# HaokunChen245/FedDAT

Measured on AMD Instinct MI355X. Metric: VQA samples/sec, ViLT-B/32 dual-adapter local step, higher is better.
Workload: dtype fp16; 1 GPU; configs[1] with fp16 operands (BASELINE.json's configs[1] string says bf16: same operand width and MFMA rate; the bf16 step is in other_operand_format with --full): ViLT-B/32 FedDAT, 1 client per MI355X, fp16 MFMA operands (dynamic loss scale, GradScaler semantics on the device, initial 2^14), fp32 accumulate / masters, batch=32/client, 384x384 synthetic + 40-token questions, MKD on; batch_per_client=32, seq_len=185, clients=1, hip_graph=True, ranks=1, hetero_steps=False

## Files before the change

feddat_amd/csrc/adapter_wgrad.hip:

```cpp
#include "common.hip.h"

namespace {

constexpr int H = 768, R = 48, NRT = 3, CW = 64;
constexpr int NCH = H / CW;
constexpr int NBLK = 10;
constexpr int PSTRIDE = R * H + R + H;

__device__ __forceinline__ void split_bf16x2(const float (&x)[8], tbf16x8& head, tbf16x8& rest) {
    typedef unsigned int u32x4_t __attribute__((ext_vector_type(4)));
    head = cvt8_tbf16(f32x4{x[0], x[1], x[2], x[3]}, f32x4{x[4], x[5], x[6], x[7]});
    const u32x4_t hp = __builtin_bit_cast(u32x4_t, head);
    float r[8];
#pragma unroll
    for (int k = 0; k < 4; ++k) {
        r[2 * k] = x[2 * k] - __uint_as_float(hp[k] << 16);
        r[2 * k + 1] = x[2 * k + 1] - __uint_as_float(hp[k] & 0xffff0000u);
    }
    rest = cvt8_tbf16(f32x4{r[0], r[1], r[2], r[3]}, f32x4{r[4], r[5], r[6], r[7]});
}

struct WgradLaunch {
    feddat_wgrad_seg seg[2];
    float* partials;
    int nseg;
};

__global__ __launch_bounds__(256, 2) void wgrad_kernel(WgradLaunch L) {
    __shared__ __attribute__((aligned(16))) float red[3][64][NRT * 4 * 4 + 4];
    const int lane = threadIdx.x & 63;
    const int wave = __builtin_amdgcn_readfirstlane(threadIdx.x >> 6);
    const int g = lane >> 4, i16 = lane & 15;
    const int blk = blockIdx.x, chunk = blockIdx.y;
    const int prob = blockIdx.z;
    const feddat_wgrad_seg& sg = L.seg[prob >> 1];
    const bool up = prob & 1;
    const float* big = up ? sg.dy : sg.x;
    const float* sm = up ? sg.z : sg.dz;
    float unscale = sg.grad_unscale != 0.0f ? sg.grad_unscale : 1.0f;
    if (sg.grad_unscale_dev) unscale *= *sg.grad_unscale_dev;
    const float alpha = (up ? sg.scale : 1.0f) * unscale;
    const int T = sg.rows;
    int tps = (T + NBLK * 4 - 1) / (NBLK * 4);
    tps = (tps + 7) & ~7;
    const int t_begin = (blk * 4 + wave) * tps;
    const int t_end = min(T, t_begin + tps);
    const int c0 = chunk * CW;

    f32x4 acc[NRT][4];
#pragma unroll
    for (int rt = 0; rt < NRT; ++rt)
#pragma unroll
        for (int v = 0; v < 4; ++v) acc[rt][v] = f32x4{0.f, 0.f, 0.f, 0.f};
    f32x4 bsum = {0.f, 0.f, 0.f, 0.f};
    float ssum[NRT] = {0.f, 0.f, 0.f};
    f32x4 braw[8];
    float sraw[8][NRT];
    const int su = NRT * i16;
    auto load_round = [&](int t0, f32x4 (&bq)[8], float (&sq)[8][NRT]) {
#pragma unroll
        for (int e = 0; e < 8; ++e) {
            const int t = t0 + 8 * g + e;
            const int tc = t < t_end ? t : 0;
            bq[e] = *reinterpret_cast<const f32x4*>(big + (size_t)tc * H + c0 + 4 * i16);
            const float* sp = sm + (size_t)tc * R + su;
#pragma unroll
            for (int rt = 0; rt < NRT; ++rt) sq[e][rt] = sp[rt];
        }
    };
    load_round(t_begin, braw, sraw);
    for (int t0 = t_begin; t0 < t_end; t0 += 32) {
        f32x4 bnext[8];
        float snext[8][NRT];
        load_round(t0 + 32, bnext, snext);
#pragma unroll
        for (int e = 0; e < 8; ++e) {
            if (t0 + 8 * g + e >= t_end) {
                braw[e] = f32x4{0.f, 0.f, 0.f, 0.f};
#pragma unroll
                for (int rt = 0; rt < NRT; ++rt) sraw[e][rt] = 0.f;
            }
            bsum = bsum + braw[e];
#pragma unroll
            for (int rt = 0; rt < NRT; ++rt) ssum[rt] += sraw[e][rt];
        }
        tbf16x8 sh[NRT], sl[NRT];
#pragma unroll
        for (int rt = 0; rt < NRT; ++rt) {
            float x[8];
#pragma unroll
            for (int e = 0; e < 8; ++e) x[e] = sraw[e][rt];
            split_bf16x2(x, sh[rt], sl[rt]);
        }
#pragma unroll
        for (int v = 0; v < 4; ++v) {
            float x[8];
#pragma unroll
            for (int e = 0; e < 8; ++e) x[e] = braw[e][v];
            tbf16x8 bh, bl;
            split_bf16x2(x, bh, bl);
#pragma unroll
            for (int rt = 0; rt < NRT; ++rt) {
                acc[rt][v] = mfma16x32_tbf16(sl[rt], bl, acc[rt][v]);
                acc[rt][v] = mfma16x32_tbf16(sl[rt], bh, acc[rt][v]);
                acc[rt][v] = mfma16x32_tbf16(sh[rt], bl, acc[rt][v]);
                acc[rt][v] = mfma16x32_tbf16(sh[rt], bh, acc[rt][v]);
            }
        }
#pragma unroll
        for (int e = 0; e < 8; ++e) {
            braw[e] = bnext[e];
#pragma unroll
            for (int rt = 0; rt < NRT; ++rt) sraw[e][rt] = snext[e][rt];
        }
    }
#pragma unroll
    for (int v = 0; v < 4; ++v) {
        bsum[v] += __shfl_xor(bsum[v], 16, 64);
        bsum[v] += __shfl_xor(bsum[v], 32, 64);
    }
#pragma unroll
    for (int rt = 0; rt < NRT; ++rt) {
        ssum[rt] += __shfl_xor(ssum[rt], 16, 64);
        ssum[rt] += __shfl_xor(ssum[rt], 32, 64);
    }
    if (wave > 0) {
        float* dst = red[wave - 1][lane];
#pragma unroll
        for (int rt = 0; rt < NRT; ++rt)
#pragma unroll
            for (int v = 0; v < 4; ++v) *reinterpret_cast<f32x4*>(dst + (rt * 4 + v) * 4) = acc[rt][v];
        if (g == 0) *reinterpret_cast<f32x4*>(dst + NRT * 16) = bsum;
    }
    __shared__ float red_s[3][NRT][16];
    if (wave > 0 && g == 0) {
#pragma unroll
        for (int rt = 0; rt < NRT; ++rt) red_s[wave - 1][rt][i16] = ssum[rt];
    }
    __syncthreads();
    if (wave != 0) return;
#pragma unroll
    for (int w = 0; w < 3; ++w) {
        const float* src = red[w][lane];
#pragma unroll
        for (int rt = 0; rt < NRT; ++rt)
#pragma unroll
            for (int v = 0; v < 4; ++v) acc[rt][v] = acc[rt][v] + *reinterpret_cast<const f32x4*>(src + (rt * 4 + v) * 4);
        if (g == 0) {
            bsum = bsum + *reinterpret_cast<const f32x4*>(src + NRT * 16);
#pragma unroll
            for (int rt = 0; rt < NRT; ++rt) ssum[rt] += red_s[w][rt][i16];
        }
    }
    float* P = L.partials + ((size_t)prob * NBLK + blk) * PSTRIDE;
#pragma unroll
    for (int rt = 0; rt < NRT; ++rt)
#pragma unroll
        for (int e = 0; e < 4; ++e) {
            const int r = NRT * (4 * g + e) + rt;
            f32x4 o = {alpha * acc[rt][0][e], alpha * acc[rt][1][e], alpha * acc[rt][2][e], alpha * acc[rt][3][e]};
            *reinterpret_cast<f32x4*>(P + (size_t)r * H + c0 + 4 * i16) = o;
        }
    if (g == 0) {
        f32x4 o = {alpha * bsum[0], alpha * bsum[1], alpha * bsum[2], alpha * bsum[3]};
        *reinterpret_cast<f32x4*>(P + R * H + R + c0 + 4 * i16) = o;
        if (chunk == 0) {
#pragma unroll
            for (int rt = 0; rt < NRT; ++rt) P[R * H + NRT * i16 + rt] = unscale * ssum[rt];
        }
    }
}

constexpr int RED_T = 384, RED_UC = 32;
constexpr int RED_UT = H / RED_UC;
constexpr int RED_DQ = (R * H + R) / 4;
constexpr int RED_DB = (RED_DQ + RED_T - 1) / RED_T;
constexpr int RED_BLOCKS = RED_UT + RED_DB + 1;
constexpr int RED_LD = R + 4;
static_assert(R * RED_UC == 4 * RED_T && H % RED_UC == 0 && (R * H) % 4 == 0 && R % 4 == 0 && H / 4 <= RED_T, "reduce tiling");

__device__ __forceinline__ f32x4 wgrad_sum_partials(const float* __restrict__ p0) {
    f32x4 p[NBLK];
#pragma unroll
    for (int b = 0; b < NBLK; ++b) p[b] = *reinterpret_cast<const f32x4*>(p0 + (size_t)b * PSTRIDE);
    f32x4 s = {0.f, 0.f, 0.f, 0.f};
#pragma unroll
    for (int b = 0; b < NBLK; ++b) s = s + p[b];
    return s;
}
__device__ __forceinline__ bool fd_nonfinite4(const f32x4 v) {
    return fd_nonfinite(v[0]) || fd_nonfinite(v[1]) || fd_nonfinite(v[2]) || fd_nonfinite(v[3]);
}

__device__ __forceinline__ bool wgrad_reduce_block(const float* __restrict__ partials, float* __restrict__ gl, int seg) {
    __shared__ __attribute__((aligned(16))) float tile[RED_UC * RED_LD];
    const float* Pd = partials + (size_t)(2 * seg) * NBLK * PSTRIDE;
    const float* Pu = partials + (size_t)(2 * seg + 1) * NBLK * PSTRIDE;
    const int blk = blockIdx.x, q = threadIdx.x;
    if (blk < RED_UT) {
        const int c0 = blk * RED_UC, r = q / (RED_UC / 4), cq = q % (RED_UC / 4);
        const f32x4 su = wgrad_sum_partials(Pu + (size_t)r * H + c0 + 4 * cq);
#pragma unroll
        for (int e = 0; e < 4; ++e) tile[(4 * cq + e) * RED_LD + r] = su[e];
        __syncthreads();
        const int c = q / (R / 4), r4 = 4 * (q % (R / 4));
        const f32x4 o = *reinterpret_cast<const f32x4*>(tile + c * RED_LD + r4);
        *reinterpret_cast<f32x4*>(gl + R * H + R + (size_t)(c0 + c) * R + r4) = o;
        return fd_nonfinite4(o);
    }
    if (blk < RED_UT + RED_DB) {
        const int i = ((blk - RED_UT) * RED_T + q) * 4;
        if (i >= R * H + R) return false;
        const f32x4 sd = wgrad_sum_partials(Pd + i);
        *reinterpret_cast<f32x4*>(gl + i) = sd;
        return fd_nonfinite4(sd);
    }
    if (q >= H / 4) return false;
    const f32x4 su = wgrad_sum_partials(Pu + R * H + R + 4 * q);
    *reinterpret_cast<f32x4*>(gl + R * H + R + H * R + 4 * q) = su;
    return fd_nonfinite4(su);
}

__global__ __launch_bounds__(RED_T) void wgrad_reduce_kernel(WgradLaunch L) {
    wgrad_reduce_block(L.partials, L.seg[blockIdx.y].grad, blockIdx.y);
}

struct WgradReduceBatch {
    float* const* grads;
    const float* partials;
    long stride;
    int nseg;
    int* nonfinite;
};
__global__ __launch_bounds__(RED_T) void wgrad_reduce_batched_kernel(WgradReduceBatch B) {
    const bool bad =
        wgrad_reduce_block(B.partials + (size_t)blockIdx.z * B.stride, B.grads[blockIdx.z * B.nseg + blockIdx.y], blockIdx.y);
    if (B.nonfinite && __ballot(bad) != 0 && (threadIdx.x & 63) == 0) atomicOr(B.nonfinite + blockIdx.y, 1);
}

}

extern "C" long feddat_adapter_wgrad_workspace_elems(int nseg) { return (long)nseg * 2 * NBLK * PSTRIDE; }

static int wgrad_launch(const feddat_wgrad_seg* segs, int nseg, float* partials, long partials_elems, int Hd, int r,
                        bool reduce_now, hipStream_t stream) {
    FD_CHECK_ARG(segs && nseg >= 1 && nseg <= 2 && partials && Hd == H && r == R);
    FD_CHECK_ARG(partials_elems >= (long)nseg * 2 * NBLK * PSTRIDE);
    WgradLaunch L;
    L.nseg = nseg;
    L.partials = partials;
    for (int s = 0; s < nseg; ++s) {
        FD_CHECK_ARG(segs[s].x && segs[s].dy && segs[s].z && segs[s].dz && segs[s].grad && segs[s].rows > 0);
        FD_CHECK_ARG(!reduce_now || (((uintptr_t)segs[s].grad | (uintptr_t)partials) & 15) == 0);
        L.seg[s] = segs[s];
    }
    if (nseg == 1) L.seg[1] = L.seg[0];
    hipLaunchKernelGGL(wgrad_kernel, dim3(NBLK, NCH, 2 * nseg), dim3(256), 0, stream, L);
    if (reduce_now) hipLaunchKernelGGL(wgrad_reduce_kernel, dim3(RED_BLOCKS, nseg), dim3(RED_T), 0, stream, L);
    FD_LAUNCH_RET();
}

extern "C" int feddat_adapter_wgrad(const feddat_wgrad_seg* segs, int nseg, float* partials, long partials_elems,
                                    int Hd, int r, hipStream_t stream) {
    return wgrad_launch(segs, nseg, partials, partials_elems, Hd, r, true, stream);
}

extern "C" int feddat_adapter_wgrad_partial(const feddat_wgrad_seg* segs, int nseg, float* partials, long partials_elems,
                                            int Hd, int r, hipStream_t stream) {
    return wgrad_launch(segs, nseg, partials, partials_elems, Hd, r, false, stream);
}

extern "C" int feddat_adapter_wgrad_reduce(float* const* grads_dev, int n, int nseg, const float* partials,
                                           long partials_stride, hipStream_t stream) {
    FD_CHECK_ARG(grads_dev && partials && n > 0 && n <= 65535 && nseg >= 1 && nseg <= 2);
    FD_CHECK_ARG(partials_stride >= (long)nseg * 2 * NBLK * PSTRIDE);
    FD_CHECK_ARG(((uintptr_t)partials & 15) == 0 && partials_stride % 4 == 0);
    hipLaunchKernelGGL(wgrad_reduce_batched_kernel, dim3(RED_BLOCKS, nseg, n), dim3(RED_T), 0, stream,
                       WgradReduceBatch{grads_dev, partials, partials_stride, nseg, nullptr});
    FD_LAUNCH_RET();
}

extern "C" int feddat_adapter_wgrad_reduce_checked(float* const* grads_dev, int n, int nseg, const float* partials,
                                                   long partials_stride, int* nonfinite, hipStream_t stream) {
    FD_CHECK_ARG(grads_dev && partials && n > 0 && n <= 65535 && nseg >= 1 && nseg <= 2 && nonfinite);
    FD_CHECK_ARG(partials_stride >= (long)nseg * 2 * NBLK * PSTRIDE);
    FD_CHECK_ARG(((uintptr_t)partials & 15) == 0 && partials_stride % 4 == 0);
    hipLaunchKernelGGL(wgrad_reduce_batched_kernel, dim3(RED_BLOCKS, nseg, n), dim3(RED_T), 0, stream,
                       WgradReduceBatch{grads_dev, partials, partials_stride, nseg, nonfinite});
    FD_LAUNCH_RET();
}
```

Before: 4894 samples/s.

## Software-pipeline adapter wgrad loads and spread block reduction across all waves

Restructures the adapter weight-gradient kernel's main loop into ping-pong register buffers. Big-operand loads for the next round are issued up front, and the small-operand loads are deferred until after the current split. Bf16 splitting of the next column tile is interleaved with the current tile's MFMAs using sched_barriers. The cross-wave reduction now has all four waves write to shared memory, and waves 1-3 each reduce and store one rank tile while wave 0 handles the bias and sum terms. This removes the serial single-wave epilogue. It also loads the device unscale factor early and disables fp contraction to keep the arithmetic identical. The costs are more registers and shared memory, which may hurt occupancy at 2 blocks per CU.

Measured after the change: 4907 samples/s (median of 6 runs). No clear change (+0.3%).

```diff
diff --git a/feddat_amd/csrc/adapter_wgrad.hip b/feddat_amd/csrc/adapter_wgrad.hip
--- a/feddat_amd/csrc/adapter_wgrad.hip
+++ b/feddat_amd/csrc/adapter_wgrad.hip
@@ -27,7 +27,8 @@
 };
 
 __global__ __launch_bounds__(256, 2) void wgrad_kernel(WgradLaunch L) {
-    __shared__ __attribute__((aligned(16))) float red[3][64][NRT * 4 * 4 + 4];
+#pragma clang fp contract(off)
+    __shared__ __attribute__((aligned(16))) float red[4][64][NRT * 4 * 4 + 4];
     const int lane = threadIdx.x & 63;
     const int wave = __builtin_amdgcn_readfirstlane(threadIdx.x >> 6);
     const int g = lane >> 4, i16 = lane & 15;
@@ -37,83 +38,100 @@
     const bool up = prob & 1;
     const float* big = up ? sg.dy : sg.x;
     const float* sm = up ? sg.z : sg.dz;
-    float unscale = sg.grad_unscale != 0.0f ? sg.grad_unscale : 1.0f;
-    if (sg.grad_unscale_dev) unscale *= *sg.grad_unscale_dev;
-    const float alpha = (up ? sg.scale : 1.0f) * unscale;
     const int T = sg.rows;
     int tps = (T + NBLK * 4 - 1) / (NBLK * 4);
     tps = (tps + 7) & ~7;
     const int t_begin = (blk * 4 + wave) * tps;
     const int t_end = min(T, t_begin + tps);
     const int c0 = chunk * CW;
-
-    f32x4 acc[NRT][4];
-#pragma unroll
-    for (int rt = 0; rt < NRT; ++rt)
-#pragma unroll
-        for (int v = 0; v < 4; ++v) acc[rt][v] = f32x4{0.f, 0.f, 0.f, 0.f};
-    f32x4 bsum = {0.f, 0.f, 0.f, 0.f};
-    float ssum[NRT] = {0.f, 0.f, 0.f};
-    f32x4 braw[8];
-    float sraw[8][NRT];
+    const float* const unscale_dev = sg.grad_unscale_dev;
+    const float unscale_dyn = *(unscale_dev ? unscale_dev : big);
+
+    f32x4 acc[NRT][4], bsum;
+    float ssum[NRT];
+    f32x4 bA[8], bB[8];
+    typedef float f32x3 __attribute__((ext_vector_type(3), aligned(4)));
+    f32x3 sq[8];
     const int su = NRT * i16;
-    auto load_round = [&](int t0, f32x4 (&bq)[8], float (&sq)[8][NRT]) {
-#pragma unroll
-        for (int e = 0; e < 8; ++e) {
-            const int t = t0 + 8 * g + e;
-            const int tc = t < t_end ? t : 0;
-            bq[e] = *reinterpret_cast<const f32x4*>(big + (size_t)tc * H + c0 + 4 * i16);
-            const float* sp = sm + (size_t)tc * R + su;
-#pragma unroll
-            for (int rt = 0; rt < NRT; ++rt) sq[e][rt] = sp[rt];
-        }
+    auto row_of = [&](int t) { return t < t_end ? t : 0; };
+    auto load_big = [&](int t0, f32x4 (&bq)[8]) {
+#pragma unroll
+        for (int e = 0; e < 8; ++e)
+            bq[e] = *reinterpret_cast<const f32x4*>(big + (size_t)row_of(t0 + 8 * g + e) * H + c0 + 4 * i16);
+        __builtin_amdgcn_sched_barrier(0);
     };
-    load_round(t_begin, braw, sraw);
-    for (int t0 = t_begin; t0 < t_end; t0 += 32) {
-        f32x4 bnext[8];
-        float snext[8][NRT];
-        load_round(t0 + 32, bnext, snext);
+    auto load_small = [&](int t0) {
+        __builtin_amdgcn_sched_barrier(0);
+#pragma unroll
+        for (int e = 0; e < 8; ++e)
+            sq[e] = *reinterpret_cast<const f32x3*>(sm + (size_t)row_of(t0 + 8 * g + e) * R + su);
+        __builtin_amdgcn_sched_barrier(0);
+    };
+    auto round = [&](int t0, f32x4 (&bq)[8], f32x4 (&bnext)[8]) {
+        load_big(t0 + 32, bnext);
 #pragma unroll
         for (int e = 0; e < 8; ++e) {
             if (t0 + 8 * g + e >= t_end) {
-                braw[e] = f32x4{0.f, 0.f, 0.f, 0.f};
-#pragma unroll
-                for (int rt = 0; rt < NRT; ++rt) sraw[e][rt] = 0.f;
+                bq[e] = f32x4{0.f, 0.f, 0.f, 0.f};
+                sq[e] = f32x3{0.f, 0.f, 0.f};
             }
-            bsum = bsum + braw[e];
-#pragma unroll
-            for (int rt = 0; rt < NRT; ++rt) ssum[rt] += sraw[e][rt];
+            bsum = bsum + bq[e];
+#pragma unroll
+            for (int rt = 0; rt < NRT; ++rt) ssum[rt] += sq[e][rt];
         }
         tbf16x8 sh[NRT], sl[NRT];
 #pragma unroll
         for (int rt = 0; rt < NRT; ++rt) {
             float x[8];
 #pragma unroll
-            for (int e = 0; e < 8; ++e) x[e] = sraw[e][rt];
+            for (int e = 0; e < 8; ++e) x[e] = sq[e][rt];
             split_bf16x2(x, sh[rt], sl[rt]);
         }
+        load_small(t0 + 32);
+        tbf16x8 bh[2], bl[2];
+        auto split_tile = [&](int v) {
+            float x[8];
+#pragma unroll
+            for (int e = 0; e < 8; ++e) x[e] = bq[e][v];
+            split_bf16x2(x, bh[v & 1], bl[v & 1]);
+        };
+        split_tile(0);
 #pragma unroll
         for (int v = 0; v < 4; ++v) {
-            float x[8];
-#pragma unroll
-            for (int e = 0; e < 8; ++e) x[e] = braw[e][v];
-            tbf16x8 bh, bl;
-            split_bf16x2(x, bh, bl);
+            __builtin_amdgcn_sched_barrier(0);
+            if (v + 1 < 4) split_tile(v + 1);
 #pragma unroll
             for (int rt = 0; rt < NRT; ++rt) {
-                acc[rt][v] = mfma16x32_tbf16(sl[rt], bl, acc[rt][v]);
-                acc[rt][v] = mfma16x32_tbf16(sl[rt], bh, acc[rt][v]);
-                acc[rt][v] = mfma16x32_tbf16(sh[rt], bl, acc[rt][v]);
-                acc[rt][v] = mfma16x32_tbf16(sh[rt], bh, acc[rt][v]);
+                acc[rt][v] = mfma16x32_tbf16(sl[rt], bl[v & 1], acc[rt][v]);
+                acc[rt][v] = mfma16x32_tbf16(sl[rt], bh[v & 1], acc[rt][v]);
+                acc[rt][v] = mfma16x32_tbf16(sh[rt], bl[v & 1], acc[rt][v]);
+                acc[rt][v] = mfma16x32_tbf16(sh[rt], bh[v & 1], acc[rt][v]);
             }
         }
-#pragma unroll
-        for (int e = 0; e < 8; ++e) {
-            braw[e] = bnext[e];
-#pragma unroll
-            for (int rt = 0; rt < NRT; ++rt) sraw[e][rt] = snext[e][rt];
-        }
-    }
+    };
+    load_big(t_begin, bA);
+    load_small(t_begin);
+#pragma unroll
+    for (int rt = 0; rt < NRT; ++rt)
+#pragma unroll
+        for (int v = 0; v < 4; ++v) acc[rt][v] = f32x4{0.f, 0.f, 0.f, 0.f};
+    bsum = f32x4{0.f, 0.f, 0.f, 0.f};
+#pragma unroll
+    for (int rt = 0; rt < NRT; ++rt) ssum[rt] = 0.f;
+    if (t_begin < t_end) {
+        int t0 = t_begin;
+        for (;;) {
+            round(t0, bA, bB);
+            t0 += 32;
+            if (t0 >= t_end) break;
+            round(t0, bB, bA);
+            t0 += 32;
+            if (t0 >= t_end) break;
+        }
+    }
+    float unscale = sg.grad_unscale != 0.0f ? sg.grad_unscale : 1.0f;
+    if (unscale_dev) unscale *= unscale_dyn;
+    const float alpha = (up ? sg.scale : 1.0f) * unscale;
 #pragma unroll
     for (int v = 0; v < 4; ++v) {
         bsum[v] += __shfl_xor(bsum[v], 16, 64);
@@ -124,13 +142,13 @@
         ssum[rt] += __shfl_xor(ssum[rt], 16, 64);
         ssum[rt] += __shfl_xor(ssum[rt], 32, 64);
     }
-    if (wave > 0) {
-        float* dst = red[wave - 1][lane];
+    {
+        float* dst = red[wave][lane];
 #pragma unroll
         for (int rt = 0; rt < NRT; ++rt)
 #pragma unroll
             for (int v = 0; v < 4; ++v) *reinterpret_cast<f32x4*>(dst + (rt * 4 + v) * 4) = acc[rt][v];
-        if (g == 0) *reinterpret_cast<f32x4*>(dst + NRT * 16) = bsum;
+        if (wave > 0 && g == 0) *reinterpret_cast<f32x4*>(dst + NRT * 16) = bsum;
     }
     __shared__ float red_s[3][NRT][16];
     if (wave > 0 && g == 0) {
@@ -138,36 +156,36 @@
         for (int rt = 0; rt < NRT; ++rt) red_s[wave - 1][rt][i16] = ssum[rt];
     }
     __syncthreads();
-    if (wave != 0) return;
-#pragma unroll
-    for (int w = 0; w < 3; ++w) {
-        const float* src = red[w][lane];
-#pragma unroll
-        for (int rt = 0; rt < NRT; ++rt)
-#pragma unroll
-            for (int v = 0; v < 4; ++v) acc[rt][v] = acc[rt][v] + *reinterpret_cast<const f32x4*>(src + (rt * 4 + v) * 4);
-        if (g == 0) {
-            bsum = bsum + *reinterpret_cast<const f32x4*>(src + NRT * 16);
-#pragma unroll
-            for (int rt = 0; rt < NRT; ++rt) ssum[rt] += red_s[w][rt][i16];
-        }
-    }
     float* P = L.partials + ((size_t)prob * NBLK + blk) * PSTRIDE;
-#pragma unroll
-    for (int rt = 0; rt < NRT; ++rt)
-#pragma unroll
-        for (int e = 0; e < 4; ++e) {
-            const int r = NRT * (4 * g + e) + rt;
-            f32x4 o = {alpha * acc[rt][0][e], alpha * acc[rt][1][e], alpha * acc[rt][2][e], alpha * acc[rt][3][e]};
-            *reinterpret_cast<f32x4*>(P + (size_t)r * H + c0 + 4 * i16) = o;
-        }
-    if (g == 0) {
+    if (wave == 0) {
+        if (g != 0) return;
+#pragma unroll
+        for (int w = 1; w < 4; ++w) {
+            bsum = bsum + *reinterpret_cast<const f32x4*>(red[w][lane] + NRT * 16);
+#pragma unroll
+            for (int rt = 0; rt < NRT; ++rt) ssum[rt] += red_s[w - 1][rt][i16];
+        }
         f32x4 o = {alpha * bsum[0], alpha * bsum[1], alpha * bsum[2], alpha * bsum[3]};
         *reinterpret_cast<f32x4*>(P + R * H + R + c0 + 4 * i16) = o;
         if (chunk == 0) {
 #pragma unroll
             for (int rt = 0; rt < NRT; ++rt) P[R * H + NRT * i16 + rt] = unscale * ssum[rt];
         }
+        return;
+    }
+    const int rt = wave - 1;
+    f32x4 a[4];
+#pragma unroll
+    for (int v = 0; v < 4; ++v) a[v] = *reinterpret_cast<const f32x4*>(red[0][lane] + (rt * 4 + v) * 4);
+#pragma unroll
+    for (int w = 1; w < 4; ++w)
+#pragma unroll
+        for (int v = 0; v < 4; ++v) a[v] = a[v] + *reinterpret_cast<const f32x4*>(red[w][lane] + (rt * 4 + v) * 4);
+#pragma unroll
+    for (int e = 0; e < 4; ++e) {
+        const int r = NRT * (4 * g + e) + rt;
+        f32x4 o = {alpha * a[0][e], alpha * a[1][e], alpha * a[2][e], alpha * a[3][e]};
+        *reinterpret_cast<f32x4*>(P + (size_t)r * H + c0 + 4 * i16) = o;
     }
 }
 
```
